# NagsTheProgrammer/WindGNN

Measured on AMD Instinct MI355X. Metric: windows/sec (fwd+bwd) 34-node seq24 GCN-GRU, higher is better.
Workload: dtype f16x3(split-fp32); 1 GPU; S=34 stations, T=24, F=13, H=102, B=4096 windows/GPU; step = forward + MSE + backward + grad all-reduce (N>1) + Adam; fp32 I/O; global_batch=4096, parallelism=dp1, math=f16x3, collective=none (one rank)

## Files before the change

### include/windgnn.h

```cpp
#ifndef WINDGNN_H
#define WINDGNN_H

#include <stddef.h>
#include <stdint.h>

#ifdef __cplusplus
extern "C" {
#endif

#define WGNN_VERSION 122

#define WGNN_STATUS_BYTES 256
#define WGNN_STATUS_ACT_RANGE 1u
#define WGNN_STATUS_WEIGHT_RANGE 2u
#define WGNN_STATUS_GRAD_NONFINITE 4u
#define WGNN_STATUS_NO_LOSS_STATS 8u

typedef enum wgnn_status {
  WGNN_OK = 0,
  WGNN_ERR_NULL = -1,
  WGNN_ERR_SHAPE = -2,
  WGNN_ERR_DTYPE = -3,
  WGNN_ERR_WORKSPACE = -4,
  WGNN_ERR_UNSUPPORTED = -5,
// ... 12 lines not shown

typedef enum wgnn_io { WGNN_IO_F32 = 0, WGNN_IO_F16 = 1, WGNN_IO_BF16 = 2 } wgnn_io;

typedef struct wgnn_dims {
  int32_t B;
  int32_t T;
  int32_t S;
  int32_t F;
  int32_t H;
  int32_t math;
  int32_t adj_format;
  int32_t nnz;
  int32_t io;
} wgnn_dims;

typedef struct wgnn_params {
  const float* conv1_weight;
  const float* conv1_bias;
  const float* conv2_weight;
  const float* conv2_bias;
  const float* w_ih;
  const float* w_hh;
  const float* b_ih;
  const float* b_hh;
  void* prepared;
} wgnn_params;

typedef struct wgnn_grads {
  float* conv1_weight;
  float* conv1_bias;
  float* conv2_weight;
  float* conv2_bias;
  float* w_ih;
  float* w_hh;
  float* b_ih;
  float* b_hh;
} wgnn_grads;

typedef struct wgnn_adam {
  wgnn_grads exp_avg;
  wgnn_grads exp_avg_sq;
  int32_t step;
  float lr, beta1, beta2, eps;
} wgnn_adam;

int wgnn_version(void);
const char* wgnn_strerror(int status);

#define WGNN_OPT_FUSED_FWD 0
#define WGNN_OPT_GG_ROLE_SPLIT 1
#define WGNN_OPT_GG_GEMM_PRIO 2
#define WGNN_OPT_BIG_GEMM 4
#define WGNN_OPT_GEMM32_FORM 5
#define WGNN_OPT_COUNT 6
int wgnn_set_option(int key, int value);
int wgnn_get_option(int key);

size_t wgnn_workspace_bytes(const wgnn_dims* d);
size_t wgnn_stash_bytes(const wgnn_dims* d);

int wgnn_fwd(const wgnn_dims* d, const float* A, const void* X , const wgnn_params* p, void* Y ,
             void* stash, void* workspace, size_t workspace_bytes, void* stream);

int wgnn_fwd_loss(const wgnn_dims* d, const float* A, const void* X, const wgnn_params* p, const void* labels,
                  void* Y, void* stash, void* workspace, size_t workspace_bytes, void* stream);

int wgnn_fwd_last(const wgnn_dims* d, const float* A, const void* X, const wgnn_params* p, float wind_min,
                  float wind_max, float* out, void* workspace, size_t workspace_bytes, void* stream);

int wgnn_fwd_state(const wgnn_dims* d, const float* A, const void* X, const wgnn_params* p, const float* h0, void* Y,
                   float* h_n, void* workspace, size_t workspace_bytes, void* stream);

size_t wgnn_state_stash_bytes(const wgnn_dims* d);
int wgnn_fwd_state_stash(const wgnn_dims* d, const float* A, const void* X, const wgnn_params* p, const float* h0, void* Y,
                         float* h_n, void* stash, void* workspace, size_t workspace_bytes, void* stream);
int wgnn_bwd_state_part(const wgnn_dims* d, const float* A, const void* X, const wgnn_params* p, const void* Y,
                        const float* dY, const float* dh_n, const void* stash, const wgnn_grads* g, float* dh0,
                        void* workspace, size_t workspace_bytes, void* stream, int part );

int wgnn_bwd(const wgnn_dims* d, const float* A, const void* X, const wgnn_params* p,
             const void* Y, const float* dY , const void* stash, const wgnn_grads* g,
             void* workspace, size_t workspace_bytes, void* stream);

int wgnn_bwd_part(const wgnn_dims* d, const float* A, const void* X, const wgnn_params* p,
                  const void* Y, const float* dY, const void* stash, const wgnn_grads* g,
                  void* workspace, size_t workspace_bytes, void* stream, int part );

int wgnn_bwd_mse_part(const wgnn_dims* d, const float* A, const void* X, const wgnn_params* p,
                      const void* Y, const void* labels , float grad_scale, float* loss,
                      const void* stash, const wgnn_grads* g, void* workspace, size_t workspace_bytes,
                      void* stream, int part );

#define WGNN_BWD_DEFER 16

#define WGNN_FINISH_ADAM_GRU 16
#define WGNN_FINISH_ADAM_CONV 32
int wgnn_finish(const wgnn_dims* d, const wgnn_params* p, const wgnn_grads* g, int which, const wgnn_adam* adam,
                void* workspace, size_t workspace_bytes, void* stream);

#define WGNN_ROWS_IH 1
#define WGNN_ROWS_HH 2
#define WGNN_ROWS_STATE 4
int wgnn_bwd_rows_align(const wgnn_dims* d);
int wgnn_bwd_rows(const wgnn_dims* d, const void* Y, const void* stash, const wgnn_grads* g, int which, int row0, int rows,
                  void* workspace, size_t workspace_bytes, void* stream);
int wgnn_finish_rows(const wgnn_dims* d, const wgnn_params* p, const wgnn_grads* g, int which, int row0, int rows,
                     const wgnn_adam* adam, void* workspace, size_t workspace_bytes, void* stream);
// ... 46 lines not shown
```

### windgnn_amd/_lib.py

```python
from __future__ import annotations

import ctypes as C
import os

_HERE = os.path.dirname(os.path.abspath(__file__))
LIB_PATH = os.environ.get("WGNN_LIB") or os.path.join(_HERE, "csrc", "libwindgnn_hip.so")

MATH_F32 = 0
MATH_F16X3 = 1
MATH_F16 = 2
MATH_F16X3G = 3
ADJ_DENSE = 0
ADJ_CSR = 1
IO_F32, IO_F16, IO_BF16 = 0, 1, 2
STEP_MAX_B = 256
STATUS_BYTES = 256
OPT_FUSED_FWD = 0
OPT_GG_ROLE_SPLIT, OPT_GG_GEMM_PRIO, OPT_BIG_GEMM, OPT_GEMM32_FORM = 1, 2, 4, 5


class Dims(C.Structure):
    _fields_ = [("B", C.c_int32), ("T", C.c_int32), ("S", C.c_int32), ("F", C.c_int32), ("H", C.c_int32),
                ("math", C.c_int32), ("adj_format", C.c_int32), ("nnz", C.c_int32), ("io", C.c_int32)]


_SLOTS = ("conv1_weight", "conv1_bias", "conv2_weight", "conv2_bias", "w_ih", "w_hh", "b_ih", "b_hh")


class Params(C.Structure):
    _fields_ = [(n, C.c_void_p) for n in _SLOTS] + [("prepared", C.c_void_p)]


class Grads(C.Structure):
    _fields_ = [(n, C.c_void_p) for n in _SLOTS]


class Adam(C.Structure):
    _fields_ = [("exp_avg", Grads), ("exp_avg_sq", Grads), ("step", C.c_int32), ("lr", C.c_float), ("beta1", C.c_float),
                ("beta2", C.c_float), ("eps", C.c_float)]


BWD_DEFER = 16
FINISH_ADAM_GRU = 16
FINISH_ADAM_CONV = 32
ROWS_IH, ROWS_HH, ROWS_STATE = 1, 2, 4


EXPORTS = {
    "wgnn_version": (C.c_int, []),
    "wgnn_strerror": (C.c_char_p, [C.c_int]),
    "wgnn_set_option": (C.c_int, [C.c_int, C.c_int]),
    "wgnn_get_option": (C.c_int, [C.c_int]),
    "wgnn_workspace_bytes": (C.c_size_t, [C.POINTER(Dims)]),
    "wgnn_stash_bytes": (C.c_size_t, [C.POINTER(Dims)]),
    "wgnn_fwd": (C.c_int, [C.POINTER(Dims), C.c_void_p, C.c_void_p, C.POINTER(Params), C.c_void_p, C.c_void_p,
                           C.c_void_p, C.c_size_t, C.c_void_p]),
    "wgnn_fwd_loss": (C.c_int, [C.POINTER(Dims), C.c_void_p, C.c_void_p, C.POINTER(Params), C.c_void_p, C.c_void_p,
                                C.c_void_p, C.c_void_p, C.c_size_t, C.c_void_p]),
    "wgnn_fwd_last": (C.c_int, [C.POINTER(Dims), C.c_void_p, C.c_void_p, C.POINTER(Params), C.c_float, C.c_float,
                                C.c_void_p, C.c_void_p, C.c_size_t, C.c_void_p]),
    "wgnn_fwd_state": (C.c_int, [C.POINTER(Dims), C.c_void_p, C.c_void_p, C.POINTER(Params), C.c_void_p, C.c_void_p,
                                 C.c_void_p, C.c_void_p, C.c_size_t, C.c_void_p]),
    "wgnn_state_stash_bytes": (C.c_size_t, [C.POINTER(Dims)]),
    "wgnn_fwd_state_stash": (C.c_int, [C.POINTER(Dims), C.c_void_p, C.c_void_p, C.POINTER(Params), C.c_void_p, C.c_void_p,
                                       C.c_void_p, C.c_void_p, C.c_void_p, C.c_size_t, C.c_void_p]),
    "wgnn_bwd_state_part": (C.c_int, [C.POINTER(Dims), C.c_void_p, C.c_void_p, C.POINTER(Params), C.c_void_p, C.c_void_p,
                                      C.c_void_p, C.c_void_p, C.POINTER(Grads), C.c_void_p, C.c_void_p, C.c_size_t,
                                      C.c_void_p, C.c_int]),
    "wgnn_bwd": (C.c_int, [C.POINTER(Dims), C.c_void_p, C.c_void_p, C.POINTER(Params), C.c_void_p, C.c_void_p,
                           C.c_void_p, C.POINTER(Grads), C.c_void_p, C.c_size_t, C.c_void_p]),
    "wgnn_bwd_part": (C.c_int, [C.POINTER(Dims), C.c_void_p, C.c_void_p, C.POINTER(Params), C.c_void_p, C.c_void_p,
# ... 102 lines not shown
```

### windgnn_amd/csrc/api.hip

```cpp
#include <atomic>
#include <cmath>
#include <cstdlib>
#include <mutex>

#include "common.h"

namespace {

inline size_t rup(size_t x, size_t a) { return (x + a - 1) / a * a; }

struct Layout {
  size_t BT, I, Ip, G3, Gp, H, Hp;
  size_t Id;
  int np_g3, np_i;
  size_t ws_GI, ws_g, ws_planes_f, ws_Ylast, ws_xtail_f, ws_xtail_b, fwd_floats;
  size_t st_g, st_gates, st_yp, stash_floats;
  size_t ws_dGI, ws_dGH, ws_dg, ws_part_ih, ws_part_hh, ws_gcnpart, ws_planes_b, ws_scales, ws_dY, bwd_floats;
  size_t prep_f, prep_b, prep_floats;
  int prep_kind;
  int sk_ih, sk_hh;
  bool x3, gen_gcn, gen_gru, g32, g32tn;
  int hq;
  int np_h;
  bool dg16;
// ... 188 lines not shown
void fill_reduce(const Layout& L, const wgnn_dims* d, const wgnn_grads* g, float* ws, int which, FinishArgs& a) {
  a.scales = ws + L.ws_scales;
  a.status = (unsigned*)ws;
  slots(*g, a.g);
  const int F = d->F;
  const int64_t n[8] = {(int64_t)F * F, F, (int64_t)F * F, F, (int64_t)L.G3 * (int64_t)L.I, (int64_t)L.G3 * (int64_t)L.H,
                        (int64_t)L.G3, (int64_t)L.G3};
  for (int t = 0; t < 8; ++t) a.n[t] = (int)n[t];
  a.I = (int)L.I;
  if (which & 4) {
    FinSeg& ih = a.ih;
    ih.partial = ws + L.ws_part_ih;
    ih.splitk = L.sk_ih;
    ih.kind = L.x3 ? 2 : 1;
    ih.Mout = ih.Mgemm = (int)L.G3; ih.Nout = (int)L.I + 1; ih.ncols = (int)L.I;
    ih.scaled = L.x3;
    FinSeg& hh = a.hh;
    hh = ih;
    hh.partial = ws + L.ws_part_hh;
    hh.splitk = L.sk_hh;
    hh.Nout = (int)L.H + 1; hh.ncols = (int)L.H;
    hh.Mgemm = L.m_hh;
    ih.pitch = L.g32tn ? gemm32_tn_pitch(ih.Nout) : ih.Nout;
    hh.pitch = L.g32tn ? gemm32_tn_pitch(hh.Nout) : hh.Nout;
    if (L.dghn) { hh.msplit = L.msplit; hh.rows1 = 2 * d->H; }
    if (L.x3) {
      pgemm_tn_geom((int)L.G3, ih.Nout, &ih.T, &ih.nNb, &ih.ntiles);
      pgemm_tn_geom(L.m_hh, hh.Nout, &hh.T, &hh.nNb, &hh.ntiles);
    }
  }
  if (which & 2) {
    a.conv_partial = ws + L.ws_gcnpart;
    a.conv_rows = L.gen_gcn ? gcn_csr_bwd_rows()
                            : (L.x3 ? gcnx_bwd_grid((int)L.BT, d->S, three_pass(d)) : gcn32_bwd_grid((int)L.BT, d->S));
  }
}

std::atomic<int> g_opt[WGNN_OPT_COUNT];
std::once_flag g_opt_once;

int env_int(const char* name, int dflt, int lo, int hi) {
  const char* e = getenv(name);
  if (!e || !e[0]) return dflt;
  char* end = nullptr;
  const long v = strtol(e, &end, 10);
  return (end == e || v < lo || v > hi) ? dflt : (int)v;
}

void init_options() {
  std::call_once(g_opt_once, [] {
    for (int k = 0; k < WGNN_OPT_COUNT; ++k) g_opt[k].store(0, std::memory_order_relaxed);
    g_opt[WGNN_OPT_FUSED_FWD].store(env_int("WGNN_FUSED_FWD", 1, 0, 2), std::memory_order_relaxed);
    g_opt[WGNN_OPT_BIG_GEMM].store(1, std::memory_order_relaxed);
  });
}

int opt(int key) {
  init_options();
  return g_opt[key].load(std::memory_order_relaxed);
}

bool known_option(int key) { return key >= 0 && key < WGNN_OPT_COUNT && key != 3; }

int check_dims(const wgnn_dims* d) {
  if (!d) return WGNN_ERR_NULL;
  if (d->B < 1 || d->T < 1 || d->S < 1 || d->H < 1) return WGNN_ERR_SHAPE;
  if (d->F != 13) return WGNN_ERR_SHAPE;
  if ((int64_t)d->B * d->T > (1 << 30)) return WGNN_ERR_SHAPE;
  if (d->math != WGNN_MATH_F32 && d->math != WGNN_MATH_F16X3 && d->math != WGNN_MATH_F16 && d->math != WGNN_MATH_F16X3G)
    return WGNN_ERR_DTYPE;
  if (d->io != WGNN_IO_F32 && d->io != WGNN_IO_F16 && d->io != WGNN_IO_BF16) return WGNN_ERR_DTYPE;
  if (d->io != WGNN_IO_F32 &&
      (d->math == WGNN_MATH_F32 || d->adj_format != WGNN_ADJ_DENSE || d->S > 64 || !grux_shape_supported(d->H)))
    return WGNN_ERR_UNSUPPORTED;
  if (d->adj_format == WGNN_ADJ_CSR) {
    if (d->nnz < 1 || (int64_t)d->nnz > (int64_t)d->S * d->S) return WGNN_ERR_SHAPE;
  } else if (d->adj_format == WGNN_ADJ_DENSE) {
    if (d->S > 64) return WGNN_ERR_UNSUPPORTED;
  } else {
    return WGNN_ERR_UNSUPPORTED;
  }
  if ((int64_t)3 * d->H * d->S * d->F >= (1ll << 31) || (int64_t)3 * d->H * d->H >= (1ll << 31)) return WGNN_ERR_SHAPE;
  if ((int64_t)d->B * d->T * d->S * d->F >= (1ll << 31) || (int64_t)d->B * d->T * 4 * d->H >= (1ll << 31))
    return WGNN_ERR_SHAPE;
  return WGNN_OK;
}

struct FwdCall {
  const float* A = nullptr;
  const void* X = nullptr;
  const float* g_in = nullptr;
  const wgnn_params* p = nullptr;
  const void* labels = nullptr;
  const float* h0 = nullptr;
  void* Y = nullptr;
  float* hn = nullptr;
  float* last = nullptr;
  float wind_min = 0.f, wind_max = 1.f;
  void* stash = nullptr;
  bool state = false, sst = false;
  void* workspace;
  size_t workspace_bytes;
  void* stream;
  FwdCall(void* ws, size_t ws_bytes, void* st) : workspace(ws), workspace_bytes(ws_bytes), stream(st) {}
};

// ... 381 lines not shown
  FinishArgs a = {};
  fill_reduce(L, d, c.g, b.ws, 2, a);
  return launch_finish(a, b.st);
}

int bwd(const wgnn_dims* d, const BwdCall& c) {
  const int which = c.part;
  if (which < 1 || which > 31 || (which & 7) == 0) return WGNN_ERR_SHAPE;
  int rc = check_dims(d);
  if (rc != WGNN_OK) return rc;
  if ((!c.dg_out && (!c.A || !c.X)) || !c.p || !c.Y || (!c.dY && !c.labels) || !c.stash || !c.g || !c.workspace)
    return WGNN_ERR_NULL;
  if (c.labels && (which & 1) && !c.loss) return WGNN_ERR_NULL;
  if (!complete(*c.g, !c.dg_out)) return WGNN_ERR_NULL;
  if (c.dg_out && (d->math != WGNN_MATH_F32 || d->io != WGNN_IO_F32 || d->adj_format != WGNN_ADJ_DENSE || which != 7))
    return WGNN_ERR_UNSUPPORTED;
  const Layout L = make_layout(d, c.sst);
  if (c.workspace_bytes < sizeof(float) * L.bwd_floats) return WGNN_ERR_WORKSPACE;
  const Bwd b{d, c, L};
  if (d->io != WGNN_IO_F32 && c.labels && (which & 1) && !(b.fused_loss && b.stats_ready)) return WGNN_ERR_UNSUPPORTED;
  if (which & 1) {
    rc = bwd_rec(b);
    if (rc != WGNN_OK) return rc;
  }
  if (which & 4) {
    rc = bwd_weights(b, WGNN_ROWS_IH | WGNN_ROWS_HH, 0, (int)L.G3);
    if (rc != WGNN_OK) return rc;
  }
  return (which & 2) ? bwd_dg(b) : WGNN_OK;
}

int rows_align(const wgnn_dims* d, const Layout& L) {
  if (!L.gen_gru || d->math == WGNN_MATH_F16) return 0;
  return L.x3 ? TN_BM : 128;
}

int check_rows(const wgnn_dims* d, const Layout& L, int which, int row0, int rows) {
  if ((which & ~(WGNN_ROWS_IH | WGNN_ROWS_HH | WGNN_ROWS_STATE)) != 0 ||
      ((which & 3) != WGNN_ROWS_IH && (which & 3) != WGNN_ROWS_HH))
    return WGNN_ERR_SHAPE;
  if (which & WGNN_ROWS_STATE) return WGNN_ERR_UNSUPPORTED;
  const int al = rows_align(d, L);
  if (al == 0) return WGNN_ERR_UNSUPPORTED;
  const int64_t end = (int64_t)row0 + rows;
  if (row0 < 0 || rows < 1 || end > (int64_t)L.G3 || row0 % al != 0 || (end % al != 0 && end != (int64_t)L.G3))
    return WGNN_ERR_SHAPE;
  return WGNN_OK;
}

}

int opt_big_gemm() { return opt(WGNN_OPT_BIG_GEMM); }
int opt_gemm32_form() { return opt(WGNN_OPT_GEMM32_FORM); }

extern "C" {

int wgnn_version(void) { return WGNN_VERSION; }

int wgnn_get_option(int key) { return known_option(key) ? opt(key) : WGNN_ERR_SHAPE; }

int wgnn_set_option(int key, int value) {
  if (!known_option(key)) return WGNN_ERR_SHAPE;
  if (key == WGNN_OPT_FUSED_FWD && (value < 0 || value > 2)) return WGNN_ERR_SHAPE;
  if ((key == WGNN_OPT_GG_ROLE_SPLIT && (value < 0 || value > 1)) || (key == WGNN_OPT_GG_GEMM_PRIO && (value < 0 || value > 3)))
    return WGNN_ERR_SHAPE;
  if (key == WGNN_OPT_BIG_GEMM && (value < 0 || value > 1)) return WGNN_ERR_SHAPE;
  if (key == WGNN_OPT_GEMM32_FORM && (value < 0 || value > 34)) return WGNN_ERR_SHAPE;
  init_options();
  return g_opt[key].exchange(value, std::memory_order_relaxed);
}

const char* wgnn_strerror(int status) {
  switch (status) {
    case WGNN_OK: return "ok";
    case WGNN_ERR_NULL: return "required pointer is NULL";
    case WGNN_ERR_SHAPE: return "invalid shape (need B,T,S,H >= 1 and F == 13)";
    case WGNN_ERR_DTYPE: return "unsupported dtype / math mode";
    case WGNN_ERR_WORKSPACE: return "workspace or stash too small";
    case WGNN_ERR_UNSUPPORTED:
      return "configuration not supported by this build (a dense adjacency needs S <= 64: pass larger graphs as CSR)";
    case WGNN_ERR_HIP: return "HIP runtime error (kernel launch failed)";
    case WGNN_ERR_RANGE:
      return "a value left fp16's range in an fp16-plane math mode (status block bits: 1 activation, 2 weight, 4 "
             "non-finite gradient): normalise the inputs or use WGNN_MATH_F32; or (bit 8) the backward was told the "
             "forward's loss statistics are in the stash but the last forward on it was not wgnn_fwd_loss";
    default: return "unknown status";
  }
}

size_t wgnn_workspace_bytes(const wgnn_dims* d) {
  if (check_dims(d) != WGNN_OK) return 0;
  Layout L = make_layout(d);
  return sizeof(float) * (L.fwd_floats > L.bwd_floats ? L.fwd_floats : L.bwd_floats);
}

size_t wgnn_stash_bytes(const wgnn_dims* d) {
  if (check_dims(d) != WGNN_OK) return 0;
  return sizeof(float) * make_layout(d).stash_floats;
}

size_t wgnn_state_stash_bytes(const wgnn_dims* d) {
  if (check_dims(d) != WGNN_OK) return 0;
  return sizeof(float) * make_layout(d, true).stash_floats;
}

size_t wgnn_prepared_bytes(const wgnn_dims* d) {
  if (check_dims(d) != WGNN_OK) return 0;
  return sizeof(float) * make_layout(d).prep_floats;
}

int wgnn_fwd(const wgnn_dims* d, const float* A, const void* X, const wgnn_params* p, void* Y, void* stash,
             void* workspace, size_t workspace_bytes, void* stream) {
  FwdCall c(workspace, workspace_bytes, stream);
  c.A = A; c.X = X; c.p = p; c.Y = Y; c.stash = stash;
  return fwd(d, c);
}

int wgnn_fwd_loss(const wgnn_dims* d, const float* A, const void* X, const wgnn_params* p, const void* labels,
                  void* Y, void* stash, void* workspace, size_t workspace_bytes, void* stream) {
  if (!labels || !stash) return WGNN_ERR_NULL;
// ... 266 lines not shown
```

### windgnn_amd/csrc/common.h

```cpp
#pragma once
#include <hip/hip_runtime.h>
#include <stdint.h>

#include "../../include/windgnn.h"

typedef float f32x4 __attribute__((ext_vector_type(4)));
typedef float f32x16 __attribute__((ext_vector_type(16)));

#define WGNN_WAVE 64

static inline int cdiv_i(int a, int b) { return (a + b - 1) / b; }
static inline size_t align_up(size_t x, size_t a) { return (x + a - 1) / a * a; }

#define WGNN_CHECK_LAUNCH()                              \
  do {                                                   \
    if (hipGetLastError() != hipSuccess) return WGNN_ERR_HIP; \
  } while (0)

__device__ __forceinline__ f32x4 mfma16(float a, float b, f32x4 c) {
  return __builtin_amdgcn_mfma_f32_16x16x4f32(a, b, c, 0, 0, 0);
}
__device__ __forceinline__ f32x16 mfma32(float a, float b, f32x16 c) {
  return __builtin_amdgcn_mfma_f32_32x32x2f32(a, b, c, 0, 0, 0);
}
// ... 84 lines not shown
                    const float* h0 = nullptr ,
                    float* hn = nullptr ,
                    size_t plane_rows = 0 );
int grux_blocks(int B);
int mse_stats_blocks();
int grux_hn(int H);
int grux_msplit(int H);
int launch_grux_bwd(int B, int T, int H, const float* Whh, const void* Y, const float* dY, const void* labels, int io,
                    const float* gates, const float* GI , int ldgi,
                    const float* scales, void* dGI_planes, void* dGHn_planes, int ldd, bool x3, const float* stat_part,
                    int64_t n_loss, float grad_scale, float* loss, float* scales_out, unsigned* status,
                    int write_lo , hipStream_t st,
                    const BwdState* state = nullptr );
#define WGNN_STATS_TAG 20261004.0f


int launch_gcn_partial_reduce(const float* partial, int nblk, float* dW1, float* db1, float* dW2, float* db2,
                              unsigned* status, hipStream_t st);
size_t gcn32_bwd_partial_floats(int ntiles);
int launch_gcn32_fwd(int ntiles, int S, const float* A, const float* X, const float* W1, const float* b1,
                     const float* W2, const float* b2, float* g, int ldg, float* xtail_scratch, hipStream_t st);
int launch_gcn32_bwd(int ntiles, int S, const float* A, const float* X, const float* W1, const float* b1,
                     const float* W2, const float* g, int ldg, const float* dg, int ld_dg, float* dW1, float* db1, float* dW2,
                     float* db2, float* partial, float* xtail_scratch, hipStream_t st);
size_t gcnx2_bwd_partial_floats(int ntiles);
int gcnx_bwd_grid(int ntiles, int S, bool x3);
int launch_gcnx2_fwd(int ntiles, int S, const float* A, const void* X, int io , const float* W1, const float* b1,
                     const float* W2, const float* b2, void* g_planes, int ldg, bool x3, unsigned* status, void* xtail_scratch,
                     hipStream_t st);
int launch_gcnx2_bwd(int ntiles, int S, const float* A, const void* X, int io, const float* W1, const float* b1,
                     const float* W2, const void* g_planes, int ldg, const void* dg, int ld_dg ,
                     bool dg16 , const float* scales, int scale_in, float* partial, bool x3,
                     void* xtail_scratch, hipStream_t st);
bool gcngi_supported(int S, int H, bool x3);
int launch_gcngi_fwd(int ntiles, int S, const float* A, const void* X, int io, const float* W1, const float* b1,
                     const float* W2, const float* b2, void* g_planes, int ldg, int stash_planes, const void* Bplanes,
                     int Np, void* GI, int ldgi, int N, bool x3, unsigned* status, void* xtail_scratch, hipStream_t st,
                     int role_split = 0, int gemm_prio = 0);
bool gcn_any_supported(int S, int Fi, int Fo);
size_t gcn_any_bwd_partial_floats(int ntiles, int Fi, int Fo);
int launch_gcn_any_fwd(int ntiles, int S, int Fi, int Fo, const float* A, const float* X, const float* W, const float* b, float* out,
                       hipStream_t st);
int launch_gcn_any_bwd(int ntiles, int S, int Fi, int Fo, const float* A, const float* X, const float* W, const float* out,
                       const float* dout, float* dW, float* db, float* dX, float* partial, hipStream_t st);
int launch_pack_g(const float* gin, size_t rows, int I, float* g, int ld, hipStream_t st);
int launch_unpack_dg(const float* dg, size_t rows, int I, int ld, float* out, hipStream_t st);
bool pgemm_nt256_wanted(int M, int N, int Kp);
int launch_pgemm_nt256(const void* Aimg_hi, const void* Aimg_lo, int M, int k0, int klen, const void* Bplanes, int Np,
                       size_t bplane, float* C, int ldc, int N, bool accumulate, hipStream_t st);
size_t pgemm_nt256_aimg_bytes(int M, int N, int Kp, int planes);
int launch_pgemm_repack_a(const void* Ahi, const void* Alo, int lda, int M, int Kp, void* img, hipStream_t st);
int opt_gemm32_form();
int opt_big_gemm();
__host__ __device__ __forceinline__ size_t bimg_off(int n, int k, int Np) {
  return ((size_t)(k >> 5) * (size_t)(Np >> 4) + (size_t)(n >> 4)) * 512 + (size_t)(((k >> 3) & 3) * 128 + (n & 15) * 8 + (k & 7));
}
int launch_split_weight2(const float* W, int R, int C, int transpose, const float* bias, int bias_col, void* planes,
                         int Rp, int Cp, unsigned* status, hipStream_t st);
int pgemm_nt_np(int N);
int pgemm_tn_tiles(int Mout, int Nout);
size_t pgemm_tn_partial_floats(int Mout, int Nout, int splitk);
size_t pgemm_nt_kpart_floats(int M, int ldc, int Kp);
int launch_pgemm_nt(const void* Ahi, const void* Alo, int lda, int M, int Kp, const void* Bplanes, int Np, float* C,
                    int ldc, int N, const float* s_out, bool x3, float* kpart, hipStream_t st, bool out16 = false,
                    void* aimg = nullptr );
int launch_pgemm_tn(const void* Ahi, const void* Alo, int lda, const void* Bhi, const void* Blo, int ldb, int shift_T,
                    int K, int splitk, float* partial, int Mout, int Nout, bool x3, const void* A2hi, const void* A2lo,
                    int lda2, int msplit, hipStream_t st, bool b_stream = false ,
                    bool per_window = false );
size_t gcn_csr_bwd_partial_floats();
int launch_gcn2_csr_fwd(int ntiles, int S, int nnz, const void* csr, const float* X, const float* W1, const float* b1,
                        const float* W2, const float* b2, float* h1, float* g, void* g_planes, size_t ldg, bool x3,
                        unsigned* status, hipStream_t st);
int launch_gcn2_csr_bwd(int ntiles, int S, int nnz, const void* csr, const float* X, const float* W2, const float* h1,
                        const float* g, const void* g_hi, size_t ldg, const float* dg, size_t ld_dg,
                        const float* scales, float* du, float* partial, float* dW1, float* db1, float* dW2, float* db2,
                        hipStream_t st);
int launch_gru_gen_fwd_x3(int B, int T, int H, const float* GI, int ldgi, const void* whh_planes, int np_g3,
                          const float* bhh, float* Y, float* gates, void* y_planes, float* gh, float* kpart, void* hc,
                          bool x3, hipStream_t st, const float* h0 = nullptr,
                          size_t plane_rows = 0 );
int launch_h0_planes(int B, int H, int Hp, const float* h0, void* hi, void* lo, hipStream_t st);
int launch_gru_gen_bwd_x3(int B, int T, int H, const void* whhT_planes, int np_h, const float* Y, const float* dY,
                          const float* gates, const float* scales, void* dgi_planes, void* dgh_planes, int ldd,
                          float* dhz, float* dhw, float* kpart, void* dc, bool x3, hipStream_t st,
                          const BwdState* state = nullptr);
int launch_gru_gen_fwd(int B, int T, int H, const float* GI, int ldgi, const float* Whh, const float* bhh, float* Y,
                       float* gates, float* gh, hipStream_t st, const float* h0 = nullptr);
int launch_gru_gen_bwd(int B, int T, int H, const float* Whh, const float* Y, const float* dY, const float* gates,
                       float* dGI, float* dGH, int ldd, float* dhz, float* dhw, hipStream_t st,
                       const BwdState* state = nullptr);
size_t gcn1_csr_bwd_ws_floats(int ntiles, int S);
int launch_gcn1_csr_fwd(int ntiles, int S, int nnz, const void* csr, const float* X, const float* W, const float* b,
                        float* out, hipStream_t st);
int launch_gcn1_csr_bwd(int ntiles, int S, int nnz, const void* csr, const float* X, const float* W, const float* out,
                        const float* dout, float* dW, float* db, float* dX, float* ws, hipStream_t st);
int launch_gcn1_fwd(int ntiles, int S, const float* A, const float* X, const float* W,
                    const float* b, float* out, hipStream_t st);
size_t gcn1_bwd_partial_floats(int ntiles);
int launch_gcn1_bwd(int ntiles, int S, const float* A, const float* X, const float* W,
                    const float* out, const float* dout, float* dW, float* db, float* dX,
                    float* partial, hipStream_t st);

int launch_gru_fwd(int B, int T, int H, const float* GI, int ldgi, const float* Whh, const float* bhh, float* Y,
                   float* gates, const float* labels, float* stat_part, float* hprev, int hq, int last_only, float y_mul,
                   float y_add, hipStream_t st, const float* h0 = nullptr, float* hn = nullptr);
// ... 82 lines not shown
```

### windgnn_amd/csrc/pgemm.hip

```cpp
#include <string>

#include "common.h"

typedef _Float16 h8 __attribute__((ext_vector_type(8)));
typedef _Float16 h4 __attribute__((ext_vector_type(4)));
typedef __fp16 fh4 __attribute__((__vector_size__(4 * sizeof(__fp16))));
typedef unsigned int u32x4 __attribute__((ext_vector_type(4)));

namespace {

constexpr int NT_BM = 192, NT_WAVES = 12;

__device__ __forceinline__ int swz16(int row) { return (4 - (row >> 2)) & 3; }
__device__ __forceinline__ int sw16_off(int row, int c) { return row * 64 + ((c ^ swz16(row)) << 4); }

__device__ __forceinline__ f32x4 mfma_q(h8 a, h8 b, f32x4 c) {
  return __builtin_amdgcn_mfma_f32_16x16x32_f16(a, b, c, 0, 0, 0);
}

constexpr int nt_a_slot(bool x3, bool alo) { return ((x3 && alo) ? 2 : 1) * NT_BM * 64; }
constexpr int nt_b_slot(int T, bool x3) { return (x3 ? 2 : 1) * 32 * T * 64; }
constexpr int nt_a_depth(int T, bool x3, bool alo) {
  return (!x3 && 3 * nt_a_slot(x3, alo) + 2 * nt_b_slot(T, x3) <= 156 * 1024) ? 3 : 2;
}
constexpr size_t nt_smem(int T, bool x3, bool alo) {
  return (size_t)nt_a_depth(T, x3, alo) * nt_a_slot(x3, alo) + 2 * (size_t)nt_b_slot(T, x3);
}

template <int T, bool X3, bool ALO, bool OUT16>
__global__ void __launch_bounds__(64 * NT_WAVES) pgemm_nt_kernel(const _Float16* __restrict__ Ahi,
                                                                const _Float16* __restrict__ Alo, int lda, int M,
                                                                int Kp, const _Float16* __restrict__ Bpl, int Np,
                                                                float* __restrict__ C, int ldc, int N,
                                                                const float* __restrict__ s_out_p, int nm, int nsl,
                                                                size_t bplane, int kc_len, int kc_first,
                                                                size_t cstride, int accumulate) {
  {
    const int k0 = (kc_first + (int)blockIdx.y) * kc_len;
    Ahi += k0;
    Alo += k0;
    Bpl += (size_t)(k0 / 32) * Np * 32;
    C += (size_t)blockIdx.y * cstride;
    Kp = min(kc_len, Kp - k0);
  }
  constexpr int BM = NT_BM, BNW = 16 * T, BN = 2 * BNW;
  constexpr int A_PL = BM * 64, B_PL = BN * 64;
  constexpr int PL = X3 ? 2 : 1;
  constexpr int PLA = (X3 && ALO) ? 2 : 1;
  constexpr int AP = BM / 16, BP = BN / 16;
  static_assert(AP == NT_WAVES, "every wave moves exactly PLA pieces of A per stage (the vmcnt below counts them)");
  constexpr int NITB = (PL * BP + NT_WAVES - 1) / NT_WAVES;
  constexpr int A_SLOT = PLA * A_PL, B_SLOT = PL * B_PL, DA = nt_a_depth(T, X3, ALO);
  extern __shared__ __attribute__((aligned(16))) char smem[];
  const int tid = threadIdx.x, lane = tid & 63;
  const int wave = __builtin_amdgcn_readfirstlane(tid >> 6);
  const int wm = wave % 6, wn = wave / 6;
  int sl, mt;
  if (nm >= 8) {
    const int grp = blockIdx.x / (8 * nsl), within = blockIdx.x % (8 * nsl);
    sl = within / 8;
    mt = grp * 8 + within % 8;
  } else {
    sl = blockIdx.x / nm;
    mt = blockIdx.x % nm;
// ... 154 lines not shown
          } else {
            const f32x4 a = *(const f32x4*)src;
            float* dst = C + (size_t)row * ldc + col;
            if (col + CW <= ldc) *(f32x4*)dst = a;
            else for (int e = 0; e < CW && col + e < N; ++e) dst[e] = a[e];
          }
        }
      }
      return;
    }
  }
  if (OUT16) {
    _Float16* Ch = (_Float16*)C;
    const bool odd = lane & 1;
#pragma unroll
    for (int j = 0; j < T; ++j) {
      const int col = n0 + BNW * wn + 16 * j + r16, colp = col & ~1;
#pragma unroll
      for (int i = 0; i < 2; ++i) {
        const f32x4 v = acc[i][j] * s_out;
        const float s0 = odd ? v[0] : v[2], s1 = odd ? v[1] : v[3];
        const float k0 = odd ? v[2] : v[0], k1 = odd ? v[3] : v[1];
        const float r0 = __builtin_bit_cast(float, __builtin_amdgcn_update_dpp(0, __builtin_bit_cast(int, s0), 0xB1, 0xF, 0xF, false));
        const float r1 = __builtin_bit_cast(float, __builtin_amdgcn_update_dpp(0, __builtin_bit_cast(int, s1), 0xB1, 0xF, 0xF, false));
        typedef float f2v __attribute__((ext_vector_type(2)));
        typedef _Float16 h2v __attribute__((ext_vector_type(2)));
        const f2v a0 = {odd ? r0 : k0, odd ? k0 : r0}, a1 = {odd ? r1 : k1, odd ? k1 : r1};
        const unsigned p0 = __builtin_bit_cast(unsigned, __builtin_convertvector(a0, h2v));
        const unsigned p1 = __builtin_bit_cast(unsigned, __builtin_convertvector(a1, h2v));
        const int row = m0 + 32 * wm + 16 * i + 4 * c4 + (odd ? 2 : 0);
        if (colp < N) {
          if (row < M) *(unsigned*)(Ch + (size_t)row * ldc + colp) = p0;
          if (row + 1 < M) *(unsigned*)(Ch + (size_t)(row + 1) * ldc + colp) = p1;
        }
      }
    }
    return;
  }
#pragma unroll
  for (int j = 0; j < T; ++j) {
    const int col = n0 + BNW * wn + 16 * j + r16;
    if (col >= N) continue;
#pragma unroll
    for (int i = 0; i < 2; ++i)
#pragma unroll
      for (int r = 0; r < 4; ++r) {
        const int row = m0 + 32 * wm + 16 * i + 4 * c4 + r;
        if (row < M) {
          float* dst = C + (size_t)row * ldc + col;
          const float v = acc[i][j][r] * s_out;
          *dst = accumulate ? *dst + v : v;
        }
      }
  }
}


__device__ __forceinline__ int tn_g(int stride32, int r) {
  const int u = stride32 & 7;
  return u == 0 ? (r & 7) : (u == 4 ? ((r >> 1) & 3) : ((r >> 2) & 1));
}

template <int T, bool X3, bool A2, bool ALO, bool PW = false>
__global__ void __launch_bounds__(64 * TN_WAVES) pgemm_tn_kernel(const _Float16* __restrict__ Ahi,
                                                                const _Float16* __restrict__ Alo, int lda,
                                                                const _Float16* __restrict__ Bhi,
                                                                const _Float16* __restrict__ Blo, int ldb,
                                                                int shift_T, int K, int kchunk,
                                                                float* __restrict__ partial, int Mout, int Nout,
                                                                int nNb, const _Float16* __restrict__ A2hi,
                                                                const _Float16* __restrict__ A2lo, int lda2,
                                                                int msplit, int b_stream) {
  constexpr int BM = TN_BM, BN = 32 * T;
  constexpr int ARB = BM * 2, BRB = BN * 2;
  constexpr int A_PL = 32 * ARB, B_PL = 32 * BRB, STAGE = 2 * A_PL + 2 * B_PL;
  constexpr int PL = X3 ? 2 : 1;
  constexpr int PLA = (X3 && ALO) ? 2 : 1;
  constexpr int AP = A_PL / 1024, BP = B_PL / 1024;
  constexpr int NPIECE = PLA * AP + PL * BP, NIT = (NPIECE + TN_WAVES - 1) / TN_WAVES;
  constexpr int ACH = ARB / 16, BCH = BRB / 16;
  extern __shared__ __attribute__((aligned(16))) char smem[];
  const int tid = threadIdx.x, lane = tid & 63;
  const int wave = __builtin_amdgcn_readfirstlane(tid >> 6);
  const int wm = wave & 3, wn = wave >> 2;
  const int z = blockIdx.x;
  const int mb = blockIdx.y / nNb, nb = blockIdx.y % nNb;
  const int m0 = mb * BM, n0 = nb * BN;
  const int kbeg = z * kchunk, kend = min(K, kbeg + kchunk);
  const int nk = kend > kbeg ? (kend - kbeg + 31) / 32 : 0;

  f32x4 acc[5][T];
#pragma unroll
  for (int i = 0; i < 5; ++i)
#pragma unroll
    for (int j = 0; j < T; ++j) acc[i][j] = f32x4{0.f, 0.f, 0.f, 0.f};

  const _Float16* base[NIT];
  int ld[NIT], dst[NIT], prow[NIT], pcol[NIT];
  bool on[NIT], isb[NIT];
#pragma unroll
  for (int it = 0; it < NIT; ++it) {
    const int p = wave + TN_WAVES * it;
    on[it] = p < NPIECE;
    const int pp = on[it] ? p : 0;
    isb[it] = pp >= PLA * AP;
    if (!isb[it]) {
// ... 161 lines not shown
                                 bias, bias_col, hi, lo, Rp, Cp, status));
  WGNN_CHECK_LAUNCH();
  return WGNN_OK;
}

__global__ void nt_ksum_kernel(const float* __restrict__ part, int nchunks, size_t n4, float* __restrict__ C) {
  const size_t i = (size_t)blockIdx.x * blockDim.x + threadIdx.x;
  if (i >= n4) return;
  f32x4 s = ((const f32x4*)part)[i];
  for (int c = 1; c < nchunks; ++c) s += ((const f32x4*)part)[(size_t)c * n4 + i];
  ((f32x4*)C)[i] = s;
}

#ifndef WGNN_NT_KC
#define WGNN_NT_KC 4096
#endif
constexpr int NT_KC = WGNN_NT_KC;
static int nt_chunks(int Kp) { return Kp > NT_KC + NT_KC / 2 ? cdiv_i(Kp, NT_KC) : 1; }
static void nt_shape(int M, int N, int Kp, bool splitk, int& nsl, int& T) {
  nsl = cdiv_i(N, 448);
  T = cdiv_i(cdiv_i(N, nsl), 32);
  const int nm = cdiv_i(M, NT_BM);
  if (nm * nsl * (splitk ? nt_chunks(Kp) : 1) < 192) {
    int want = cdiv_i(256, nm);
    if (want > cdiv_i(N, 32)) want = cdiv_i(N, 32);
    T = cdiv_i(cdiv_i(N, want), 32);
    nsl = cdiv_i(N, 32 * T);
  }
}
size_t pgemm_nt_kpart_floats(int M, int ldc, int Kp) { return nt_chunks(Kp) > 1 ? (size_t)nt_chunks(Kp) * M * ldc : 0; }
int pgemm_nt_np(int N) { return cdiv_i(N, 32) * 32 + 448 - 32; }

template <int T>
static int launch_nt_t(const void* Ahi, const void* Alo, int lda, int M, int Kp, const void* Bplanes, int Np, float* C,
                       int ldc, int N, const float* s_out, bool x3, int nsl, float* kpart, bool out16, hipStream_t st) {
  const bool alo = Alo != nullptr;
  const int nm = cdiv_i(M, NT_BM);
  const int grid = (nm >= 8 ? cdiv_i(nm, 8) * 8 : nm) * nsl;
  constexpr size_t smem3 = nt_smem(T, true, true), smem2 = nt_smem(T, true, false), smem1 = nt_smem(T, false, true);
  const size_t smem = x3 ? (alo ? smem3 : smem2) : smem1;
  static std::atomic<unsigned long long> done{0}, done16{0}, done2{0}, done2h{0}, done16h{0};
  if (ensure_dyn_smem((const void*)pgemm_nt_kernel<T, false, true, true>, smem1, done16h) != WGNN_OK) return WGNN_ERR_HIP;
  if (ensure_dyn_smem((const void*)pgemm_nt_kernel<T, true, true, false>, smem3, done) != WGNN_OK) return WGNN_ERR_HIP;
  if (ensure_dyn_smem((const void*)pgemm_nt_kernel<T, true, false, false>, smem2, done2) != WGNN_OK) return WGNN_ERR_HIP;
  if (ensure_dyn_smem((const void*)pgemm_nt_kernel<T, true, false, true>, smem2, done2h) != WGNN_OK) return WGNN_ERR_HIP;
  if (ensure_dyn_smem((const void*)pgemm_nt_kernel<T, false, true, false>, smem1, done16) != WGNN_OK) return WGNN_ERR_HIP;
  static const std::string name = "pgemm_nt_kernel<" + std::to_string(T) + ">", name16 = "pgemm_nt_kernel<" + std::to_string(T) + ",f16>",
                           name2 = "pgemm_nt_kernel<" + std::to_string(T) + ",x2>";
  const int nchunks = (out16 && !x3) ? 1 : nt_chunks(Kp), kc_len = nchunks > 1 ? NT_KC : Kp;
  const size_t bplane = (size_t)Np * Kp;
  const bool split = kpart && nchunks > 1;
  const int nlaunch = split ? 1 : nchunks;
  if (out16 && ((x3 && alo) || nchunks > 1 || (ldc & 1))) return WGNN_ERR_UNSUPPORTED;
  for (int c = 0; c < nlaunch; ++c) {
    const dim3 g(grid, split ? nchunks : 1);
    float* out = split ? kpart : C;
    const size_t cstride = split ? (size_t)M * ldc : 0;
    const double kk = split ? Kp : (Kp - c * kc_len < kc_len ? Kp - c * kc_len : kc_len);
    const double fl = 2.0 * M * (double)N * kk;
    const double by = (x3 && alo ? 4.0 : 2.0) * (double)M * kk + (x3 ? 4.0 : 2.0) * (double)Np * kk +
                      (out16 ? 2.0 : 4.0) * (double)M * N * (split ? nchunks : (c > 0 ? 2 : 1));
    if (x3 && alo)
      PROF_LAUNCH(name.c_str(), fl, by, st,
                  hipLaunchKernelGGL((pgemm_nt_kernel<T, true, true, false>), g, dim3(64 * NT_WAVES), smem, st, (const _Float16*)Ahi,
                                     (const _Float16*)Alo, lda, M, Kp, (const _Float16*)Bplanes, Np, out, ldc, N, s_out,
                                     nm, nsl, bplane, kc_len, c, cstride, c > 0 ? 1 : 0));
    else if (x3 && out16)
      PROF_LAUNCH(name2.c_str(), fl, by, st,
                  hipLaunchKernelGGL((pgemm_nt_kernel<T, true, false, true>), g, dim3(64 * NT_WAVES), smem, st, (const _Float16*)Ahi,
                                     (const _Float16*)Ahi, lda, M, Kp, (const _Float16*)Bplanes, Np, out, ldc, N, s_out,
                                     nm, nsl, bplane, kc_len, c, cstride, 0));
    else if (x3)
      PROF_LAUNCH(name2.c_str(), fl, by, st,
                  hipLaunchKernelGGL((pgemm_nt_kernel<T, true, false, false>), g, dim3(64 * NT_WAVES), smem, st, (const _Float16*)Ahi,
                                     (const _Float16*)Ahi, lda, M, Kp, (const _Float16*)Bplanes, Np, out, ldc, N, s_out,
                                     nm, nsl, bplane, kc_len, c, cstride, c > 0 ? 1 : 0));
    else if (out16)
      PROF_LAUNCH(name16.c_str(), fl, by, st,
                  hipLaunchKernelGGL((pgemm_nt_kernel<T, false, true, true>), g, dim3(64 * NT_WAVES), smem, st, (const _Float16*)Ahi,
                                     (const _Float16*)Ahi, lda, M, Kp, (const _Float16*)Bplanes, Np, out, ldc, N, s_out,
                                     nm, nsl, bplane, kc_len, c, cstride, 0));
    else
      PROF_LAUNCH(name16.c_str(), fl, by, st,
                  hipLaunchKernelGGL((pgemm_nt_kernel<T, false, true, false>), g, dim3(64 * NT_WAVES), smem, st, (const _Float16*)Ahi,
                                     (const _Float16*)Alo, lda, M, Kp, (const _Float16*)Bplanes, Np, out, ldc, N, s_out,
                                     nm, nsl, bplane, kc_len, c, cstride, c > 0 ? 1 : 0));
    WGNN_CHECK_LAUNCH();
  }
  if (split) {
    if (((size_t)M * ldc) % 4 != 0) return WGNN_ERR_SHAPE;
    const size_t n4 = (size_t)M * ldc / 4;
    PROF_LAUNCH("nt_ksum_kernel", 0.0, 16.0 * n4 * (nchunks + 1), st,
                hipLaunchKernelGGL(nt_ksum_kernel, dim3((unsigned)((n4 + 255) / 256)), dim3(256), 0, st, kpart, nchunks, n4,
                                   C));
    WGNN_CHECK_LAUNCH();
  }
  return WGNN_OK;
}

int launch_pgemm_nt(const void* Ahi, const void* Alo, int lda, int M, int Kp, const void* Bplanes, int Np, float* C,
                    int ldc, int N, const float* s_out, bool x3, float* kpart, hipStream_t st, bool out16, void* aimg) {
  if (x3 && !out16 && !kpart && !s_out && aimg && pgemm_nt256_wanted(M, N, Kp) && Kp % 32 == 0 && lda % 8 == 0 &&
      Np >= cdiv_i(N, 256) * 256 && opt_big_gemm()) {
    const int nchunks = nt_chunks(Kp), kc_len = nchunks > 1 ? NT_KC : Kp;
    int rc = launch_pgemm_repack_a(Ahi, Alo, lda, M, Kp, aimg, st);
    if (rc != WGNN_OK) return rc;
// ... 115 lines not shown
```

Before: 5.488 million windows/s.

## Add persistent NT GEMM kernel that prefetches next tile's first K-slice

Adds a persistent variant of the split-fp16 NT GEMM. Its grid is capped at 256 workgroups, and each block loops over output tiles in a grouped order. While it computes the last K step of one tile, it issues the DMA for the next tile's first K slice, so load latency is hidden across tile boundaries and launch and tail costs are reduced. The kernel is enabled by default through a new option and applies only to single-chunk fp32-output x3 calls. It drops the generality of the earlier kernel, including accumulate and multi-chunk support, and persistence may cost parallelism when the tile count is small.

```diff
diff --git a/include/windgnn.h b/include/windgnn.h
--- a/include/windgnn.h
+++ b/include/windgnn.h
@@ -88,7 +88,8 @@
 #define WGNN_OPT_GG_GEMM_PRIO 2
 #define WGNN_OPT_BIG_GEMM 4
 #define WGNN_OPT_GEMM32_FORM 5
-#define WGNN_OPT_COUNT 6
+#define WGNN_OPT_NT_FORM 6
+#define WGNN_OPT_COUNT 7
 int wgnn_set_option(int key, int value);
 int wgnn_get_option(int key);
 
diff --git a/windgnn_amd/_lib.py b/windgnn_amd/_lib.py
--- a/windgnn_amd/_lib.py
+++ b/windgnn_amd/_lib.py
@@ -17,6 +17,7 @@
 STATUS_BYTES = 256
 OPT_FUSED_FWD = 0
 OPT_GG_ROLE_SPLIT, OPT_GG_GEMM_PRIO, OPT_BIG_GEMM, OPT_GEMM32_FORM = 1, 2, 4, 5
+OPT_NT_FORM = 6
 
 
 class Dims(C.Structure):
diff --git a/windgnn_amd/csrc/api.hip b/windgnn_amd/csrc/api.hip
--- a/windgnn_amd/csrc/api.hip
+++ b/windgnn_amd/csrc/api.hip
@@ -264,6 +264,7 @@
     for (int k = 0; k < WGNN_OPT_COUNT; ++k) g_opt[k].store(0, std::memory_order_relaxed);
     g_opt[WGNN_OPT_FUSED_FWD].store(env_int("WGNN_FUSED_FWD", 1, 0, 2), std::memory_order_relaxed);
     g_opt[WGNN_OPT_BIG_GEMM].store(1, std::memory_order_relaxed);
+    g_opt[WGNN_OPT_NT_FORM].store(1, std::memory_order_relaxed);
   });
 }
 
@@ -751,6 +752,7 @@
 
 int opt_big_gemm() { return opt(WGNN_OPT_BIG_GEMM); }
 int opt_gemm32_form() { return opt(WGNN_OPT_GEMM32_FORM); }
+int opt_nt_form() { return opt(WGNN_OPT_NT_FORM); }
 
 extern "C" {
 
@@ -765,6 +767,7 @@
     return WGNN_ERR_SHAPE;
   if (key == WGNN_OPT_BIG_GEMM && (value < 0 || value > 1)) return WGNN_ERR_SHAPE;
   if (key == WGNN_OPT_GEMM32_FORM && (value < 0 || value > 34)) return WGNN_ERR_SHAPE;
+  if (key == WGNN_OPT_NT_FORM && (value < 0 || value > 1)) return WGNN_ERR_SHAPE;
   init_options();
   return g_opt[key].exchange(value, std::memory_order_relaxed);
 }
diff --git a/windgnn_amd/csrc/common.h b/windgnn_amd/csrc/common.h
--- a/windgnn_amd/csrc/common.h
+++ b/windgnn_amd/csrc/common.h
@@ -160,6 +160,7 @@
 int launch_pgemm_repack_a(const void* Ahi, const void* Alo, int lda, int M, int Kp, void* img, hipStream_t st);
 int opt_gemm32_form();
 int opt_big_gemm();
+int opt_nt_form();
 __host__ __device__ __forceinline__ size_t bimg_off(int n, int k, int Np) {
   return ((size_t)(k >> 5) * (size_t)(Np >> 4) + (size_t)(n >> 4)) * 512 + (size_t)(((k >> 3) & 3) * 128 + (n & 15) * 8 + (k & 7));
 }
diff --git a/windgnn_amd/csrc/pgemm.hip b/windgnn_amd/csrc/pgemm.hip
--- a/windgnn_amd/csrc/pgemm.hip
+++ b/windgnn_amd/csrc/pgemm.hip
@@ -10,6 +10,7 @@
 namespace {
 
 constexpr int NT_BM = 192, NT_WAVES = 12;
+constexpr int NT_CUS = 256;
 
 __device__ __forceinline__ int swz16(int row) { return (4 - (row >> 2)) & 3; }
 __device__ __forceinline__ int sw16_off(int row, int c) { return row * 64 + ((c ^ swz16(row)) << 4); }
@@ -270,6 +271,155 @@
           *dst = accumulate ? *dst + v : v;
         }
       }
+  }
+}
+
+template <int T, bool ALO>
+__global__ void __launch_bounds__(64 * NT_WAVES) pgemm_nt_pers_kernel(const _Float16* __restrict__ Ahi,
+                                                                     const _Float16* __restrict__ Alo, int lda, int M,
+                                                                     int Kp, const _Float16* __restrict__ Bpl, int Np,
+                                                                     float* __restrict__ C, int ldc, int N,
+                                                                     const float* __restrict__ s_out_p, int nm, int nsl,
+                                                                     size_t bplane, int ntiles) {
+  constexpr int BM = NT_BM, BNW = 16 * T, BN = 2 * BNW;
+  constexpr int A_PL = BM * 64, B_PL = BN * 64;
+  constexpr int PLA = ALO ? 2 : 1;
+  constexpr int BP = BN / 16;
+  static_assert(BM / 16 == NT_WAVES, "every wave moves exactly PLA pieces of A per stage");
+  static_assert(nt_a_depth(T, true, ALO) == 2, "two-slot rings");
+  constexpr int NITB = (2 * BP + NT_WAVES - 1) / NT_WAVES;
+  constexpr int A_SLOT = PLA * A_PL, B_SLOT = 2 * B_PL;
+  extern __shared__ __attribute__((aligned(16))) char smem[];
+  const int tid = threadIdx.x, lane = tid & 63;
+  const int wave = __builtin_amdgcn_readfirstlane(tid >> 6);
+  const int wm = wave % 6, wn = wave / 6;
+  const float s_out = s_out_p ? s_out_p[1] : 1.f;
+  const int nk = Kp / 32;
+  const int r16 = lane & 15, c4 = lane >> 4;
+  const int prow = lane >> 2, ppos = lane & 3;
+  const int chunk = 8 * (ppos ^ swz16(prow));
+  typedef __attribute__((address_space(3))) void lds_void;
+  typedef __attribute__((address_space(1))) const void glb_void;
+  char* const ringA = smem;
+  char* const ringB = smem + 2 * A_SLOT;
+
+  auto tile_at = [&](int t, int& mt, int& sl) {
+    if (nm >= 8) {
+      const int grp = t / (8 * nsl), within = t % (8 * nsl);
+      sl = within / 8;
+      mt = grp * 8 + within % 8;
+    } else {
+      sl = t / nm;
+      mt = t % nm;
+    }
+  };
+  auto next_tile = [&](int t, int& mt, int& sl) {
+    for (; t < ntiles; t += (int)gridDim.x) {
+      tile_at(t, mt, sl);
+      if (mt < nm) break;
+    }
+    return t;
+  };
+
+  const char* baseA = nullptr;
+  const char* baseB = nullptr;
+  unsigned offA = 0;
+  const unsigned offB = lane * 16;
+  const ptrdiff_t lo_A = (const char*)Alo - (const char*)Ahi;
+  auto set_src = [&](int m0, int n0) {
+    const int rb = min(m0 + 16 * wave, M - 1);
+    baseA = (const char*)(Ahi + (size_t)rb * lda);
+    offA = (unsigned)(min(prow, M - 1 - rb) * lda + chunk) * 2;
+    baseB = (const char*)(Bpl + (size_t)(n0 / 16) * 512);
+  };
+  auto uni = [](const char* p) {
+    const unsigned long long v = (unsigned long long)p;
+    const unsigned lo = __builtin_amdgcn_readfirstlane((unsigned)v), hi = __builtin_amdgcn_readfirstlane((unsigned)(v >> 32));
+    return (const char*)(((unsigned long long)hi << 32) | lo);
+  };
+  auto dma = [&](int slot, int kt) {
+#pragma unroll
+    for (int pl = 0; pl < PLA; ++pl)
+      __builtin_amdgcn_global_load_lds((glb_void*)(uni(baseA + pl * lo_A + (size_t)64 * kt) + offA),
+                                       (lds_void*)(ringA + slot * A_SLOT + pl * A_PL + wave * 1024), 16, 0, 0);
+#pragma unroll
+    for (int it = 0; it < NITB; ++it) {
+      const int q = wave + NT_WAVES * it;
+      if (q < 2 * BP)
+        __builtin_amdgcn_global_load_lds(
+            (glb_void*)(uni(baseB + ((size_t)(q / BP) * bplane + (size_t)(q % BP) * 512 + (size_t)Np * 32 * kt) * 2) + offB),
+            (lds_void*)(ringB + slot * B_SLOT + (q / BP) * B_PL + (q % BP) * 1024), 16, 0, 0);
+    }
+  };
+
+  f32x4 acc[2][T];
+  const int a_off0 = sw16_off(32 * wm + r16, c4), a_off1 = a_off0 + 16 * 64;
+  const int b_off = T * wn * 1024 + lane * 16;
+  auto compute = [&](const char* curA, const char* curB) {
+    const char* Ah = curA;
+    const char* Al = curA + A_PL;
+    const char* Bh = curB + b_off;
+    const char* Bl = Bh + B_PL;
+    h8 ah[2], al[2];
+    ah[0] = *(const h8*)(Ah + a_off0);
+    ah[1] = *(const h8*)(Ah + a_off1);
+    al[0] = ah[0];
+    al[1] = ah[1];
+    if (ALO) {
+      al[0] = *(const h8*)(Al + a_off0);
+      al[1] = *(const h8*)(Al + a_off1);
+    }
+#pragma unroll
+    for (int j = 0; j < T; ++j) {
+      const h8 bh = *(const h8*)(Bh + j * 1024);
+      const h8 bl = *(const h8*)(Bl + j * 1024);
+#pragma unroll
+      for (int i = 0; i < 2; ++i) {
+        if (ALO) acc[i][j] = mfma_q(bh, al[i], acc[i][j]);
+        acc[i][j] = mfma_q(bl, ah[i], acc[i][j]);
+      }
+#pragma unroll
+      for (int i = 0; i < 2; ++i) acc[i][j] = mfma_q(bh, ah[i], acc[i][j]);
+    }
+  };
+
+  int mt, sl;
+  int tile = next_tile((int)blockIdx.x, mt, sl);
+  if (tile >= ntiles) return;
+  set_src(mt * BM, sl * BN);
+  dma(0, 0);
+  int slot = 0;
+  for (;;) {
+    const int m0 = mt * BM, n0 = sl * BN;
+    const int nxt = next_tile(tile + (int)gridDim.x, mt, sl);
+#pragma unroll
+    for (int i = 0; i < 2; ++i)
+#pragma unroll
+      for (int j = 0; j < T; ++j) acc[i][j] = f32x4{0.f, 0.f, 0.f, 0.f};
+    for (int kt = 0; kt < nk; ++kt) {
+      asm volatile("s_waitcnt vmcnt(0)" ::: "memory");
+      __builtin_amdgcn_s_barrier();
+      if (kt + 1 < nk) {
+        dma(slot ^ 1, kt + 1);
+      } else if (nxt < ntiles) {
+        set_src(mt * BM, sl * BN);
+        dma(slot ^ 1, 0);
+      }
+      compute(ringA + slot * A_SLOT, ringB + slot * B_SLOT);
+      slot ^= 1;
+    }
+#pragma unroll
+    for (int i = 0; i < 2; ++i) {
+      const int row = m0 + 32 * wm + 16 * i + r16;
+      if (row < M) {
+        float* dst = C + (size_t)row * ldc + n0 + BNW * wn + 4 * c4;
+#pragma unroll
+        for (int j = 0; j < T; ++j)
+          if (n0 + BNW * wn + 16 * j + 4 * c4 < N) *(f32x4*)(dst + 16 * j) = acc[i][j] * s_out;
+      }
+    }
+    if (nxt >= ntiles) break;
+    tile = nxt;
   }
 }
 
@@ -537,6 +687,30 @@
   const bool split = kpart && nchunks > 1;
   const int nlaunch = split ? 1 : nchunks;
   if (out16 && ((x3 && alo) || nchunks > 1 || (ldc & 1))) return WGNN_ERR_UNSUPPORTED;
+  if (x3 && !out16 && !kpart && nchunks == 1 && Kp >= 32 && N <= ldc && ldc % 4 == 0 && ((size_t)C & 15) == 0 &&
+      opt_nt_form() == 1) {
+    static std::atomic<unsigned long long> donep{0}, donep2{0};
+    static const std::string pname = "pgemm_nt_pers_kernel<" + std::to_string(T) + ">",
+                             pname2 = "pgemm_nt_pers_kernel<" + std::to_string(T) + ",x2>";
+    const int pgrid = grid < NT_CUS ? grid : NT_CUS;
+    const double fl = 2.0 * M * (double)N * Kp;
+    const double by = (alo ? 4.0 : 2.0) * (double)M * Kp + 4.0 * (double)Np * Kp + 4.0 * (double)M * N;
+    if (alo) {
+      if (ensure_dyn_smem((const void*)pgemm_nt_pers_kernel<T, true>, smem3, donep) != WGNN_OK) return WGNN_ERR_HIP;
+      PROF_LAUNCH(pname.c_str(), fl, by, st,
+                  hipLaunchKernelGGL((pgemm_nt_pers_kernel<T, true>), dim3(pgrid), dim3(64 * NT_WAVES), smem3, st,
+                                     (const _Float16*)Ahi, (const _Float16*)Alo, lda, M, Kp, (const _Float16*)Bplanes, Np, C, ldc,
+                                     N, s_out, nm, nsl, bplane, grid));
+    } else {
+      if (ensure_dyn_smem((const void*)pgemm_nt_pers_kernel<T, false>, smem2, donep2) != WGNN_OK) return WGNN_ERR_HIP;
+      PROF_LAUNCH(pname2.c_str(), fl, by, st,
+                  hipLaunchKernelGGL((pgemm_nt_pers_kernel<T, false>), dim3(pgrid), dim3(64 * NT_WAVES), smem2, st,
+                                     (const _Float16*)Ahi, (const _Float16*)Ahi, lda, M, Kp, (const _Float16*)Bplanes, Np, C, ldc,
+                                     N, s_out, nm, nsl, bplane, grid));
+    }
+    WGNN_CHECK_LAUNCH();
+    return WGNN_OK;
+  }
   for (int c = 0; c < nlaunch; ++c) {
     const dim3 g(grid, split ? nchunks : 1);
     float* out = split ? kpart : C;
```

Result: no change. 5.517 million windows/s, median of 2 (+0.5%).
